# ddemidov/amgcl

Measured on AMD Instinct MI355X. Metric: setup+solve time (s) & iterations to 1e-6, 3D Poisson 512^3, lower is better.
Workload: dtype fp64; 1 GPU; model=3D Poisson 512^3 (7-point stencil), unknowns=134217728, solver=cg, precond=smoothed_aggregation AMG + SPAI0, iters=16, parallelism=single GPU

## Files before the change

### amgcl_amd/csrc/hip/setup.hip

```cpp

#include <hip/hip_runtime.h>

#include <cstdint>

#include "amg_kernels.h"

#define WAVE 64

static inline int nblk(int64_t work, int block = 256, int cap = 4096) {
    int64_t b = (work + block - 1) / block;
    return (int)(b < 1 ? 1 : (b > cap ? cap : b));
}

template <int LANES, int SLOTS>
__device__ __forceinline__ void lds_bitonic(int *k, double *v, int lane) {
    for (int size = 2; size <= SLOTS; size <<= 1) {
        for (int strd = size >> 1; strd > 0; strd >>= 1) {
            __builtin_amdgcn_s_waitcnt(0);
            __builtin_amdgcn_wave_barrier();
            for (int t = lane; t < SLOTS / 2; t += LANES) {
                int i = ((t / strd) * strd * 2) + (t % strd);
                int j = i + strd;
                bool up = ((i & size) == 0);
                int ki = k[i], kj = k[j];
                if ((ki > kj) == up) {
                    k[i] = kj;
                    k[j] = ki;
                    double tv = v[i];
                    v[i] = v[j];
                    v[j] = tv;
                }
            }
        }
    }
    __builtin_amdgcn_s_waitcnt(0);
    __builtin_amdgcn_wave_barrier();
}

__device__ __forceinline__ uint64_t agg_key_d(int i) {
    uint32_t x = (uint32_t)i;
    x ^= x >> 16; x *= 0x7feb352dU; x ^= x >> 15; x *= 0x846ca68bU; x ^= x >> 16;
    return ((uint64_t)x << 32) | (uint32_t)i;
}

#define SETUP_SW 4

__global__ void diag_k(int64_t n, const int *__restrict__ ptr, const int *__restrict__ col,
                       const double *__restrict__ val, double *__restrict__ d) {
    int64_t tid = (int64_t)blockIdx.x * blockDim.x + threadIdx.x;
    int lane = (int)(tid & (SETUP_SW - 1));
    int64_t i = tid / SETUP_SW;
    int64_t stride = ((int64_t)gridDim.x * blockDim.x) / SETUP_SW;
    for (; i < n; i += stride) {
        double v = 0.0;
        for (int j = ptr[i] + lane; j < ptr[i + 1]; j += SETUP_SW)
            if (col[j] == (int)i) v = val[j];
#pragma unroll
        for (int off = SETUP_SW / 2; off > 0; off >>= 1)
            v += __shfl_down(v, off, SETUP_SW);
        if (lane == 0) d[i] = v;
    }
}

__global__ void strong_k(int64_t n, const int *__restrict__ ptr, const int *__restrict__ col,
                         const double *__restrict__ val, const double *__restrict__ d,
                         double eps2, uint8_t *__restrict__ S) {
    int64_t tid = (int64_t)blockIdx.x * blockDim.x + threadIdx.x;
    int lane = (int)(tid & (SETUP_SW - 1));
    int64_t i = tid / SETUP_SW;
    int64_t stride = ((int64_t)gridDim.x * blockDim.x) / SETUP_SW;
    for (; i < n; i += stride) {
        double edi = eps2 * d[i];
        for (int j = ptr[i] + lane; j < ptr[i + 1]; j += SETUP_SW) {
            int c = col[j];
            double v = val[j];
            S[j] = (c != (int)i) && (edi * d[c] < v * v);
        }
    }
}

__global__ void spai0_k(int64_t n, const int *__restrict__ ptr, const int *__restrict__ col,
                        const double *__restrict__ val, double *__restrict__ m) {
    int64_t tid = (int64_t)blockIdx.x * blockDim.x + threadIdx.x;
    int lane = (int)(tid & (SETUP_SW - 1));
    int64_t i = tid / SETUP_SW;
    int64_t stride = ((int64_t)gridDim.x * blockDim.x) / SETUP_SW;
    for (; i < n; i += stride) {
        double num = 0.0, den = 0.0;
        for (int j = ptr[i] + lane; j < ptr[i + 1]; j += SETUP_SW) {
            double v = val[j];
            den += v * v;
            if (col[j] == (int)i) num = v;
        }
#pragma unroll
        for (int off = SETUP_SW / 2; off > 0; off >>= 1) {
            den += __shfl_down(den, off, SETUP_SW);
            num += __shfl_down(num, off, SETUP_SW);
        }
        if (lane == 0) m[i] = den > 0.0 ? num / den : 0.0;
    }
}

extern "C" int amg_setup_diag(int64_t n, const int *ptr, const int *col, const double *val,
                              double *d, hipStream_t s) {
    diag_k<<<nblk(n * SETUP_SW), 256, 0, s>>>(n, ptr, col, val, d);
    return (int)hipGetLastError();
}
extern "C" int amg_setup_strong(int64_t n, const int *ptr, const int *col, const double *val,
                                const double *d, double eps2, uint8_t *S, hipStream_t s) {
    strong_k<<<nblk(n * SETUP_SW), 256, 0, s>>>(n, ptr, col, val, d, eps2, S);
    return (int)hipGetLastError();
}
extern "C" int amg_setup_spai0(int64_t n, const int *ptr, const int *col, const double *val,
                               double *m, hipStream_t s) {
    spai0_k<<<nblk(n * SETUP_SW), 256, 0, s>>>(n, ptr, col, val, m);
    return (int)hipGetLastError();
}

__global__ void gersh_k(int64_t n, const int *__restrict__ ptr, const int *__restrict__ col,
                        const double *__restrict__ val, int scale, double *__restrict__ out) {
    __shared__ double lds[4];
    int64_t i = (int64_t)blockIdx.x * blockDim.x + threadIdx.x;
    int64_t stride = (int64_t)gridDim.x * blockDim.x;
    double m = 0.0;
    for (; i < n; i += stride) {
        double s = 0.0, dia = 1.0;
        for (int j = ptr[i]; j < ptr[i + 1]; ++j) {
            s += fabs(val[j]);
            if (col[j] == (int)i) dia = fabs(val[j]);
        }
        if (scale && dia > 0.0) s /= dia;
        if (s > m) m = s;
    }
#pragma unroll
    for (int off = 32; off > 0; off >>= 1) {
        double o = __shfl_down(m, off, 64);
        if (o > m) m = o;
    }
    int wid = threadIdx.x / 64, lane = threadIdx.x & 63;
    if (lane == 0) lds[wid] = m;
    __syncthreads();
    if (threadIdx.x == 0) {
        double bm = fmax(fmax(lds[0], lds[1]), fmax(lds[2], lds[3]));
        unsigned long long *o = (unsigned long long *)out;
        unsigned long long cur = *o;
        while (__longlong_as_double((long long)cur) < bm) {
            unsigned long long next = (unsigned long long)__double_as_longlong(bm);
            unsigned long long old = atomicCAS(o, cur, next);
            if (old == cur) break;
            cur = old;
        }
    }
}

extern "C" int amg_gershgorin(int64_t n, const int *ptr, const int *col, const double *val,
                              int scale, double *out, hipStream_t s) {
    hipMemsetAsync(out, 0, sizeof(double), s);
    gersh_k<<<nblk(n, 256, 1024), 256, 0, s>>>(n, ptr, col, val, scale, out);
    return (int)hipGetLastError();
}

#define SCAN_BLOCK 1024

__global__ void scan_block_k(int64_t n, const int *__restrict__ in, int *__restrict__ out,
                             int *__restrict__ sums) {
    __shared__ int lds[SCAN_BLOCK];
    int64_t base = (int64_t)blockIdx.x * SCAN_BLOCK;
    int t = threadIdx.x;
    lds[t] = (base + t < n) ? in[base + t] : 0;
    __syncthreads();
    for (int off = 1; off < SCAN_BLOCK; off <<= 1) {
        int v = (t >= off) ? lds[t - off] : 0;
        __syncthreads();
        lds[t] += v;
        __syncthreads();
    }
    if (base + t < n) out[base + t] = lds[t];
    if (t == SCAN_BLOCK - 1 && sums) sums[blockIdx.x] = lds[t];
}

__global__ void scan_add_k(int64_t n, int *__restrict__ out, const int *__restrict__ sums) {
    int64_t base = (int64_t)blockIdx.x * SCAN_BLOCK;
    int t = threadIdx.x;
    if (blockIdx.x > 0 && base + t < n) out[base + t] += sums[blockIdx.x - 1];
}

static int scan_i32_device(int *a, int64_t n, hipStream_t s) {
    if (n <= 0) return 0;
    int64_t nblocks = (n + SCAN_BLOCK - 1) / SCAN_BLOCK;
    if (nblocks == 1) {
        scan_block_k<<<1, SCAN_BLOCK, 0, s>>>(n, a, a, nullptr);
        return (int)hipGetLastError();
    }
    int *sums = nullptr;
    int rc = (int)hipMallocAsync((void **)&sums, nblocks * sizeof(int), s);
    if (rc) return rc;
    scan_block_k<<<nblocks, SCAN_BLOCK, 0, s>>>(n, a, a, sums);
    rc = scan_i32_device(sums, nblocks, s);
    if (rc) return rc;
    scan_add_k<<<nblocks, SCAN_BLOCK, 0, s>>>(n, a, sums);
    hipFreeAsync(sums, s);
    return (int)hipGetLastError();
}

extern "C" int amg_scan_i32(int *a, int64_t n, hipStream_t s) {
    return scan_i32_device(a, n, s);
}

__global__ void agg_init_k(int64_t n, const int *__restrict__ ptr, const uint8_t *__restrict__ S,
                           int *__restrict__ id) {
    int64_t i = (int64_t)blockIdx.x * blockDim.x + threadIdx.x;
    int64_t stride = (int64_t)gridDim.x * blockDim.x;
    for (; i < n; i += stride) {
        int st = -2;
        for (int j = ptr[i]; j < ptr[i + 1]; ++j)
            if (S[j]) { st = -1; break; }
        id[i] = st;
    }
}

#define AGG_FOREACH(i)                                                              int64_t _t = (int64_t)blockIdx.x * blockDim.x + threadIdx.x;                    int64_t _stride = (int64_t)gridDim.x * blockDim.x;                              for (; _t < nwork; _t += _stride)                                                   if (int64_t i = (list ? (int64_t)list[_t] : _t); true)

__global__ void agg_clear_near_k(int64_t nwork, const int *__restrict__ list,
                                 uint8_t *__restrict__ near) {
    AGG_FOREACH(i) near[i] = 0;
}

__global__ void agg_flag_k(int64_t nwork, const int *__restrict__ list,
                           const uint8_t *__restrict__ near, int *__restrict__ flags) {
    AGG_FOREACH(i) flags[_t] = near[i] ? 1 : 0;
}

__global__ void agg_scatter_list_k(int64_t nwork, const int *__restrict__ list,
                                   const uint8_t *__restrict__ near,
                                   const int *__restrict__ flags_scanned,
                                   int *__restrict__ out) {
    AGG_FOREACH(i) if (near[i]) out[flags_scanned[_t] - 1] = (int)i;
}

__global__ void agg_m1_k(int64_t nwork, const int *__restrict__ list,
                         const int *__restrict__ ptr, const int *__restrict__ col,
                         const uint8_t *__restrict__ S, const int *__restrict__ id,
                         const uint8_t *__restrict__ near, uint64_t *__restrict__ m1) {
    AGG_FOREACH(i) {
        if (!near[i]) {
            m1[i] = 0;
            continue;
        }
        uint64_t m = (id[i] == -1) ? agg_key_d((int)i) : 0;
        for (int j = ptr[i]; j < ptr[i + 1]; ++j) {
            if (!S[j]) continue;
            int c = col[j];
            if (id[c] == -1) {
                uint64_t k = agg_key_d(c);
                if (k > m) m = k;
            }
        }
        m1[i] = m;
    }
}

__global__ void agg_near_k(int64_t nwork, const int *__restrict__ list,
                           const int *__restrict__ ptr, const int *__restrict__ col,
                           const uint8_t *__restrict__ S, const int *__restrict__ id,
                           uint8_t *__restrict__ near) {
    AGG_FOREACH(i) {
        if (id[i] == -1) {
            near[i] = 1;
            for (int j = ptr[i]; j < ptr[i + 1]; ++j)
                if (S[j]) near[col[j]] = 1;
        }
    }
}

__global__ void agg_roots_k(int64_t nwork, const int *__restrict__ list,
                            const int *__restrict__ ptr, const int *__restrict__ col,
                            const uint8_t *__restrict__ S, int *__restrict__ id,
                            const uint64_t *__restrict__ m1, uint8_t *__restrict__ newroot) {
    AGG_FOREACH(i) {
        newroot[i] = 0;
        if (id[i] != -1) continue;
        uint64_t key = agg_key_d((int)i);
        uint64_t m2 = m1[i];
        for (int j = ptr[i]; j < ptr[i + 1] && m2 <= key; ++j) {
            if (!S[j]) continue;
            uint64_t v = m1[col[j]];
            if (v > m2) m2 = v;
        }
        if (m2 == key) {
            id[i] = (int)i;
            newroot[i] = 1;
        }
    }
}

__global__ void agg_claim_k(int64_t nwork, const int *__restrict__ list,
                            const int *__restrict__ ptr, const int *__restrict__ col,
                            const uint8_t *__restrict__ S, int *__restrict__ id,
                            uint8_t *__restrict__ prov, const uint8_t *__restrict__ newroot) {
    AGG_FOREACH(i) {
        if (!newroot[i]) continue;
        for (int j = ptr[i]; j < ptr[i + 1]; ++j) {
            int c = col[j];
            if (!S[j]) continue;
            if (id[c] == -1 || prov[c]) {
                id[c] = (int)i;
                prov[c] = 0;
            }
        }
    }
}

__global__ void agg_adopt_mark_k(int64_t nwork, const int *__restrict__ list,
                                 const int *__restrict__ ptr,
                                 const int *__restrict__ col, const uint8_t *__restrict__ S,
                                 const int *__restrict__ id, const uint8_t *__restrict__ prov,
                                 int *__restrict__ choice) {
    AGG_FOREACH(i) {
        if (id[i] != -1) continue;
        uint64_t best = 0;
        int root = -1;
        for (int j = ptr[i]; j < ptr[i + 1]; ++j) {
            int c = col[j];
            if (!S[j] || c == (int)i) continue;
            if (id[c] >= 0 && !prov[c]) {
                uint64_t k = agg_key_d(id[c]);
                if (k > best) { best = k; root = id[c]; }
            }
        }
        choice[i] = root;
    }
}

__global__ void agg_adopt_commit_k(int64_t nwork, const int *__restrict__ list,
                                   int *__restrict__ id,
                                   uint8_t *__restrict__ prov,
                                   const int *__restrict__ choice,
                                   int *__restrict__ remaining) {
    int my_remaining = 0;
    AGG_FOREACH(i) {
        if (id[i] != -1) continue;
        int root = choice[i];
        if (root >= 0) {
            id[i] = root;
            prov[i] = 1;
        } else {
            ++my_remaining;
        }
    }
#pragma unroll
    for (int off = WAVE / 2; off > 0; off >>= 1)
        my_remaining += __shfl_down(my_remaining, off, WAVE);
    if ((threadIdx.x & (WAVE - 1)) == 0 && my_remaining)
        atomicAdd(remaining, my_remaining);
}

__global__ void agg_mark_roots_k(int64_t n, const int *__restrict__ id, int *__restrict__ mark) {
    int64_t i = (int64_t)blockIdx.x * blockDim.x + threadIdx.x;
    int64_t stride = (int64_t)gridDim.x * blockDim.x;
    for (; i < n; i += stride) mark[i] = (id[i] == (int)i) ? 1 : 0;
}

__global__ void agg_relabel_k(int64_t n, int *__restrict__ id, const int *__restrict__ mark) {
    int64_t i = (int64_t)blockIdx.x * blockDim.x + threadIdx.x;
    int64_t stride = (int64_t)gridDim.x * blockDim.x;
    for (; i < n; i += stride)
        if (id[i] >= 0) id[i] = mark[id[i]] - 1;
}

extern "C" int amg_agg_init(int64_t n, const int *ptr, const uint8_t *S, int *id, hipStream_t s) {
    agg_init_k<<<nblk(n), 256, 0, s>>>(n, ptr, S, id);
    return (int)hipGetLastError();
}
static int agg_round_impl(int64_t nwork, const int *list, const int *ptr,
                          const int *col, const uint8_t *S, int *id, uint8_t *prov,
                          uint64_t *m1, uint8_t *newroot, uint8_t *near,
                          int *remaining, hipStream_t s) {
    if (list)
        agg_clear_near_k<<<nblk(nwork), 256, 0, s>>>(nwork, list, near);
    else
        (void)hipMemsetAsync(near, 0, nwork, s);
    agg_near_k<<<nblk(nwork), 256, 0, s>>>(nwork, list, ptr, col, S, id, near);
    agg_m1_k<<<nblk(nwork), 256, 0, s>>>(nwork, list, ptr, col, S, id, near, m1);
    agg_roots_k<<<nblk(nwork), 256, 0, s>>>(nwork, list, ptr, col, S, id, m1, newroot);
    agg_claim_k<<<nblk(nwork), 256, 0, s>>>(nwork, list, ptr, col, S, id, prov, newroot);
    agg_adopt_mark_k<<<nblk(nwork), 256, 0, s>>>(nwork, list, ptr, col, S, id, prov,
                                                 (int *)m1);
    agg_adopt_commit_k<<<nblk(nwork), 256, 0, s>>>(nwork, list, id, prov, (int *)m1,
                                                   remaining);
    return (int)hipGetLastError();
}

extern "C" int amg_agg_round(int64_t n, const int *ptr, const int *col, const uint8_t *S,
                             int *id, uint8_t *prov, uint64_t *m1, uint8_t *newroot,
                             uint8_t *near, int *remaining, hipStream_t s) {
    return agg_round_impl(n, nullptr, ptr, col, S, id, prov, m1, newroot, near,
                          remaining, s);
}
extern "C" int amg_agg_run(int64_t n, const int *ptr, const int *col, const uint8_t *S,
                           int *id, uint8_t *prov, uint64_t *m1, uint8_t *newroot,
                           uint8_t *near, int *remaining, int sync_stride,
                           int max_rounds, int *rounds_out, int *lists,
                           hipStream_t s) {
    int *h_rem = nullptr;
    hipError_t e = hipHostMalloc((void **)&h_rem, 2 * sizeof(int),
                                 hipHostMallocDefault);
    if (e != hipSuccess) return (int)e;
    int *L[2] = {lists, lists ? lists + n : nullptr};
    int cur = -1;
    int64_t nwork = n;
    int64_t last_rem = n;
    int first_cround = -1;
    int rc = 0;
    bool done = false;
    int round = 0;
    for (; round < max_rounds; ++round) {
        e = hipMemsetAsync(remaining, 0, sizeof(int), s);
        if (e != hipSuccess) { rc = (int)e; break; }
        const int *list = cur < 0 ? nullptr : L[cur];
        if (list)
            agg_clear_near_k<<<nblk(nwork), 256, 0, s>>>(nwork, list, near);
        else
            (void)hipMemsetAsync(near, 0, n, s);
        agg_near_k<<<nblk(nwork), 256, 0, s>>>(nwork, list, ptr, col, S, id, near);
        if (lists && last_rem * 4 < n &&
            (first_cround < 0 || (round - first_cround) % 4 == 0)) {
            int nxt = cur < 0 ? 0 : 1 - cur;
            int *F = lists + 2 * n;
            agg_flag_k<<<nblk(nwork), 256, 0, s>>>(nwork, list, near, F);
            rc = scan_i32_device(F, nwork, s);
            if (rc) break;
            agg_scatter_list_k<<<nblk(nwork), 256, 0, s>>>(nwork, list, near, F,
                                                           L[nxt]);
            e = hipMemcpyAsync(h_rem + 1, F + (nwork - 1), sizeof(int),
                               hipMemcpyDeviceToHost, s);
            if (e == hipSuccess) e = hipStreamSynchronize(s);
            if (e != hipSuccess) { rc = (int)e; break; }
            if (h_rem[1] > 0 && h_rem[1] < nwork) {
                cur = nxt;
                nwork = h_rem[1];
            }
            if (first_cround < 0) first_cround = round;
        }
        const int *list2 = cur < 0 ? nullptr : L[cur];
        agg_m1_k<<<nblk(nwork), 256, 0, s>>>(nwork, list2, ptr, col, S, id, near, m1);
        agg_roots_k<<<nblk(nwork), 256, 0, s>>>(nwork, list2, ptr, col, S, id, m1,
                                                newroot);
        agg_claim_k<<<nblk(nwork), 256, 0, s>>>(nwork, list2, ptr, col, S, id, prov,
                                                newroot);
        agg_adopt_mark_k<<<nblk(nwork), 256, 0, s>>>(nwork, list2, ptr, col, S, id,
                                                     prov, (int *)m1);
        agg_adopt_commit_k<<<nblk(nwork), 256, 0, s>>>(nwork, list2, id, prov,
                                                       (int *)m1, remaining);
        rc = (int)hipGetLastError();
        if (rc) break;
        if (round % sync_stride == sync_stride - 1 || round > 8) {
            e = hipMemcpyAsync(h_rem, remaining, sizeof(int), hipMemcpyDeviceToHost, s);
            if (e == hipSuccess) e = hipStreamSynchronize(s);
            if (e != hipSuccess) { rc = (int)e; break; }
            if (*h_rem == 0) { done = true; break; }
            last_rem = *h_rem;
        }
    }
    (void)hipHostFree(h_rem);
    if (rc) return rc;
    if (!done) return 9999;
    if (rounds_out) *rounds_out = round + 1;
    return 0;
}

extern "C" int amg_agg_renumber(int64_t n, int *id, int *mark, hipStream_t s) {
    agg_mark_roots_k<<<nblk(n), 256, 0, s>>>(n, id, mark);
    int rc = scan_i32_device(mark, n, s);
    if (rc) return rc;
    agg_relabel_k<<<nblk(n), 256, 0, s>>>(n, id, mark);
    return (int)hipGetLastError();
}

#define PROW_MAX 56
#define PSLOTS 64
#define PMASK (PSLOTS - 1)
#define PGRP 8

__global__ void psmooth_count_k(int64_t n, const int *__restrict__ ptr,
                                const int *__restrict__ col, const uint8_t *__restrict__ S,
                                const int *__restrict__ id, int *__restrict__ cnt,
                                int *__restrict__ overflow) {
    __shared__ int keys[32][PSLOTS];
    int gid = threadIdx.x / PGRP;
    int lane = threadIdx.x & (PGRP - 1);
    int64_t i = ((int64_t)blockIdx.x * blockDim.x + threadIdx.x) / PGRP;
    int64_t stride = ((int64_t)gridDim.x * blockDim.x) / PGRP;
    int *tk = keys[gid];
    for (; i < n; i += stride) {
        for (int t = lane; t < PSLOTS; t += PGRP) tk[t] = -1;
        __builtin_amdgcn_s_waitcnt(0);
        __builtin_amdgcn_wave_barrier();
        int inserted = 0;
        bool ovf = false;
        for (int j = ptr[i] + lane; j < ptr[i + 1] && !ovf; j += PGRP) {
            int c = col[j];
            if (c != (int)i && !S[j]) continue;
            int a = id[c];
            if (a < 0) continue;
            uint32_t h = ((uint32_t)a * 2654435761u) & PMASK;
            int probes = 0;
            while (true) {
                int old = atomicCAS(&tk[h], -1, a);
                if (old == -1) { ++inserted; break; }
                if (old == a) break;
                h = (h + 1) & PMASK;
                if (++probes >= PSLOTS) { ovf = true; break; }
            }
        }
        if (ovf) atomicAdd(overflow, 1);
#pragma unroll
        for (int off = PGRP / 2; off > 0; off >>= 1)
            inserted += __shfl_down(inserted, off, PGRP);
        if (lane == 0) {
            if (inserted > PROW_MAX) atomicAdd(overflow, 1);
            cnt[i] = inserted;
        }
        __builtin_amdgcn_wave_barrier();
    }
}

__global__ void psmooth_fill_k(int64_t n, const int *__restrict__ ptr,
                               const int *__restrict__ col, const double *__restrict__ val,
                               const uint8_t *__restrict__ S, const int *__restrict__ id,
                               double omega, const int *__restrict__ pptr,
                               int *__restrict__ pcol, double *__restrict__ pval) {
    __shared__ int keys[32][PSLOTS];
    __shared__ double vals[32][PSLOTS];
    int gid = threadIdx.x / PGRP;
    int lane = threadIdx.x & (PGRP - 1);
    int64_t i = ((int64_t)blockIdx.x * blockDim.x + threadIdx.x) / PGRP;
    int64_t stride = ((int64_t)gridDim.x * blockDim.x) / PGRP;
    int *tk = keys[gid];
    double *tv = vals[gid];
    for (; i < n; i += stride) {
        for (int t = lane; t < PSLOTS; t += PGRP) {
            tk[t] = -1;
            tv[t] = 0.0;
        }
        double dia = 0.0;
        for (int j = ptr[i] + lane; j < ptr[i + 1]; j += PGRP)
            if (col[j] == (int)i || !S[j]) dia += val[j];
#pragma unroll
        for (int off = PGRP / 2; off > 0; off >>= 1)
            dia += __shfl_down(dia, off, PGRP);
        dia = __shfl(dia, (threadIdx.x & ~(PGRP - 1)) & 63, 64);
        if (dia != 0.0) dia = -omega / dia;
        __builtin_amdgcn_s_waitcnt(0);
        __builtin_amdgcn_wave_barrier();
        for (int j = ptr[i] + lane; j < ptr[i + 1]; j += PGRP) {
            int c = col[j];
            if (c != (int)i && !S[j]) continue;
            int a = id[c];
            if (a < 0) continue;
            double v = (c == (int)i) ? (1.0 - omega) : dia * val[j];
            uint32_t h = ((uint32_t)a * 2654435761u) & PMASK;
            while (true) {
                int old = atomicCAS(&tk[h], -1, a);
                if (old == -1 || old == a) {
                    atomicAdd(&tv[h], v);
                    break;
                }
                h = (h + 1) & PMASK;
            }
        }
        __builtin_amdgcn_s_waitcnt(0);
        __builtin_amdgcn_wave_barrier();
        int mine = 0;
        for (int t = lane; t < PSLOTS; t += PGRP)
            if (tk[t] != -1) ++mine;
        int off = mine;
#pragma unroll
        for (int d = 1; d < PGRP; d <<= 1) {
            int v = __shfl_up(off, d, PGRP);
            if (lane >= d) off += v;
        }
        off -= mine;
        int base = (i == 0) ? 0 : pptr[i - 1];
        int h2 = base + off;
        for (int t = lane; t < PSLOTS; t += PGRP)
            if (tk[t] != -1) {
                pcol[h2] = tk[t];
                pval[h2] = tv[t];
                ++h2;
            }
        __builtin_amdgcn_wave_barrier();
    }
}

__global__ void ptent_count_k(int64_t n, const int *__restrict__ id, int *__restrict__ cnt) {
    int64_t i = (int64_t)blockIdx.x * blockDim.x + threadIdx.x;
    int64_t stride = (int64_t)gridDim.x * blockDim.x;
    for (; i < n; i += stride) cnt[i] = id[i] >= 0 ? 1 : 0;
}

__global__ void ptent_fill_k(int64_t n, const int *__restrict__ id, const int *__restrict__ pptr,
                             int *__restrict__ pcol, double *__restrict__ pval) {
    int64_t i = (int64_t)blockIdx.x * blockDim.x + threadIdx.x;
    int64_t stride = (int64_t)gridDim.x * blockDim.x;
    for (; i < n; i += stride) {
        if (id[i] < 0) continue;
        int base = (i == 0) ? 0 : pptr[i - 1];
        pcol[base] = id[i];
        pval[base] = 1.0;
    }
}

extern "C" int amg_psmooth_count(int64_t n, const int *ptr, const int *col, const uint8_t *S,
                                 const int *id, int *cnt, int *overflow, hipStream_t s) {
    psmooth_count_k<<<nblk(n * PGRP), 256, 0, s>>>(n, ptr, col, S, id, cnt, overflow);
    return (int)hipGetLastError();
}
extern "C" int amg_psmooth_fill(int64_t n, const int *ptr, const int *col, const double *val,
                                const uint8_t *S, const int *id, double omega,
                                const int *pptr_scanned, int *pcol, double *pval,
                                hipStream_t s) {
    psmooth_fill_k<<<nblk(n * PGRP), 256, 0, s>>>(n, ptr, col, val, S, id, omega,
                                                  pptr_scanned, pcol, pval);
    return (int)hipGetLastError();
}
extern "C" int amg_ptent_count(int64_t n, const int *id, int *cnt, hipStream_t s) {
    ptent_count_k<<<nblk(n), 256, 0, s>>>(n, id, cnt);
    return (int)hipGetLastError();
}
extern "C" int amg_ptent_fill(int64_t n, const int *id, const int *pptr_scanned, int *pcol,
                              double *pval, hipStream_t s) {
    ptent_fill_k<<<nblk(n), 256, 0, s>>>(n, id, pptr_scanned, pcol, pval);
    return (int)hipGetLastError();
}

__global__ void tcount_k(int64_t nnz, const int *__restrict__ col, int *__restrict__ tcnt) {
    int64_t j = (int64_t)blockIdx.x * blockDim.x + threadIdx.x;
    int64_t stride = (int64_t)gridDim.x * blockDim.x;
    for (; j < nnz; j += stride) atomicAdd(&tcnt[col[j]], 1);
}

__global__ void tscatter_k(int64_t n, const int *__restrict__ ptr, const int *__restrict__ col,
                           const double *__restrict__ val, int *__restrict__ cursor,
                           int *__restrict__ tcol, double *__restrict__ tval) {
    int64_t i = (int64_t)blockIdx.x * blockDim.x + threadIdx.x;
    int64_t stride = (int64_t)gridDim.x * blockDim.x;
    for (; i < n; i += stride) {
        for (int j = ptr[i]; j < ptr[i + 1]; ++j) {
            int c = col[j];
            int h = atomicAdd(&cursor[c], 1);
            tcol[h] = (int)i;
            tval[h] = val[j];
        }
    }
}

__global__ void sort_rows_k(int64_t n, const int *__restrict__ ptr_scanned,
                            int *__restrict__ col, double *__restrict__ val) {
    int64_t i = (int64_t)blockIdx.x * blockDim.x + threadIdx.x;
    int64_t stride = (int64_t)gridDim.x * blockDim.x;
    for (; i < n; i += stride) {
        int b = (i == 0) ? 0 : ptr_scanned[i - 1];
        int e = ptr_scanned[i];
        for (int k = b + 1; k < e; ++k) {
            int ck = col[k];
            double vk = val[k];
            int m = k;
            while (m > b && col[m - 1] > ck) {
                col[m] = col[m - 1];
                val[m] = val[m - 1];
                --m;
            }
            col[m] = ck;
            val[m] = vk;
        }
    }
}

extern "C" int amg_transpose_count(int64_t nnz, const int *col, int *tcnt, hipStream_t s) {
    tcount_k<<<nblk(nnz), 256, 0, s>>>(nnz, col, tcnt);
    return (int)hipGetLastError();
}
extern "C" int amg_transpose_scatter(int64_t n, const int *ptr, const int *col,
                                     const double *val, int *cursor, int *tcol, double *tval,
                                     hipStream_t s) {
    tscatter_k<<<nblk(n), 256, 0, s>>>(n, ptr, col, val, cursor, tcol, tval);
    return (int)hipGetLastError();
}
extern "C" int amg_sort_rows(int64_t n, const int *ptr_scanned, int *col, double *val,
                             hipStream_t s) {
    sort_rows_k<<<nblk(n), 256, 0, s>>>(n, ptr_scanned, col, val);
    return (int)hipGetLastError();
}

#define HSLOTS 512
#define HMASK (HSLOTS - 1)
#define SGRP 8
#define SSLOTS 128
#define SSMASK (SSLOTS - 1)
#define SGSMALL 96

__global__ void spgemm_ub_k(int64_t an, const int *__restrict__ aptr,
                            const int *__restrict__ acol, const int *__restrict__ bptr,
                            int *__restrict__ ub) {
    int64_t i = (int64_t)blockIdx.x * blockDim.x + threadIdx.x;
    int64_t stride = (int64_t)gridDim.x * blockDim.x;
    for (; i < an; i += stride) {
        int u = 0;
        for (int ja = aptr[i]; ja < aptr[i + 1]; ++ja) {
            int ca = acol[ja];
            u += bptr[ca + 1] - bptr[ca];
        }
        ub[i] = u;
    }
}

template <int SLOTS>
__global__ void spgemm_count_small_k(int64_t an, const int *__restrict__ aptr,
                                     const int *__restrict__ acol,
                                     const int *__restrict__ bptr,
                                     const int *__restrict__ bcol,
                                     const int *__restrict__ ub, int *__restrict__ cnt,
                                     int ub_lo, int ub_hi) {
    __shared__ int keys[32][SLOTS];
    constexpr int MASK = SLOTS - 1;
    int gid = threadIdx.x / SGRP;
    int lane = threadIdx.x & (SGRP - 1);
    int64_t row = ((int64_t)blockIdx.x * blockDim.x + threadIdx.x) / SGRP;
    int64_t stride = ((int64_t)gridDim.x * blockDim.x) / SGRP;
    int *tk = keys[gid];
    for (; row < an; row += stride) {
        int u = ub[row];
        if (u <= ub_lo || u > ub_hi) continue;
        for (int t = lane; t < SLOTS; t += SGRP) tk[t] = -1;
        __builtin_amdgcn_s_waitcnt(0);
        __builtin_amdgcn_wave_barrier();
        int inserted = 0;
        for (int ja = aptr[row]; ja < aptr[row + 1]; ++ja) {
            int ca = acol[ja];
            for (int jb = bptr[ca] + lane; jb < bptr[ca + 1]; jb += SGRP) {
                int key = bcol[jb];
                uint32_t h = ((uint32_t)key * 2654435761u) & MASK;
                while (true) {
                    int old = atomicCAS(&tk[h], -1, key);
                    if (old == -1) { ++inserted; break; }
                    if (old == key) break;
                    h = (h + 1) & MASK;
                }
            }
        }
#pragma unroll
        for (int off = SGRP / 2; off > 0; off >>= 1)
            inserted += __shfl_down(inserted, off, SGRP);
        if (lane == 0) cnt[row] = inserted;
        __builtin_amdgcn_wave_barrier();
    }
}

template <int SLOTS>
__global__ void spgemm_fill_small_k(int64_t an, const int *__restrict__ aptr,
                                    const int *__restrict__ acol,
                                    const double *__restrict__ aval,
                                    const int *__restrict__ bptr,
                                    const int *__restrict__ bcol,
                                    const double *__restrict__ bval,
                                    const int *__restrict__ ub,
                                    const int *__restrict__ cptr_scanned,
                                    int *__restrict__ ccol, double *__restrict__ cval,
                                    int do_sort, int len_lo, int len_hi) {
    __shared__ int keys[32][SLOTS];
    __shared__ double vals[32][SLOTS];
    constexpr int SMASK_S = SLOTS - 1;
    int gid = threadIdx.x / SGRP;
    int lane = threadIdx.x & (SGRP - 1);
    int64_t row = ((int64_t)blockIdx.x * blockDim.x + threadIdx.x) / SGRP;
    int64_t stride = ((int64_t)gridDim.x * blockDim.x) / SGRP;
    int *tk = keys[gid];
    double *tv = vals[gid];
    for (; row < an; row += stride) {
        if (ub[row] > SGSMALL) continue;
        int base = (row == 0) ? 0 : cptr_scanned[row - 1];
        int len = cptr_scanned[row] - base;
        if (len <= len_lo || len > len_hi) continue;
        for (int t = lane; t < SLOTS; t += SGRP) {
            tk[t] = -1;
            tv[t] = 0.0;
        }
        __builtin_amdgcn_s_waitcnt(0);
        __builtin_amdgcn_wave_barrier();
        for (int ja = aptr[row]; ja < aptr[row + 1]; ++ja) {
            int ca = acol[ja];
            double va = aval[ja];
            for (int jb = bptr[ca] + lane; jb < bptr[ca + 1]; jb += SGRP) {
                int key = bcol[jb];
                double v = va * bval[jb];
                uint32_t h = ((uint32_t)key * 2654435761u) & SMASK_S;
                while (true) {
                    int old = atomicCAS(&tk[h], -1, key);
                    if (old == -1 || old == key) {
                        atomicAdd(&tv[h], v);
                        break;
                    }
                    h = (h + 1) & SMASK_S;
                }
            }
        }
        __builtin_amdgcn_s_waitcnt(0);
        __builtin_amdgcn_wave_barrier();
        if (do_sort) {
            for (int t = lane; t < SLOTS; t += SGRP)
                if (tk[t] == -1) tk[t] = 0x7fffffff;
            lds_bitonic<SGRP, SLOTS>(tk, tv, lane);
            for (int t = lane; t < len; t += SGRP) {
                ccol[base + t] = tk[t];
                cval[base + t] = tv[t];
            }
        } else {
            int mine = 0;
            for (int t = lane; t < SLOTS; t += SGRP)
                if (tk[t] != -1) ++mine;
            int off = mine;
#pragma unroll
            for (int d = 1; d < SGRP; d <<= 1) {
                int v = __shfl_up(off, d, SGRP);
                if (lane >= d) off += v;
            }
            off -= mine;
            int h = base + off;
            for (int t = lane; t < SLOTS; t += SGRP)
                if (tk[t] != -1) {
                    ccol[h] = tk[t];
                    cval[h] = tv[t];
                    ++h;
                }
        }
        __builtin_amdgcn_wave_barrier();
    }
}

#define BIGROW 256

__device__ __forceinline__ int pfx_find(const int *pfx, int len, int t) {
    int lo = 0, hi = len;
    while (hi - lo > 1) {
        int mid = (lo + hi) >> 1;
        if (pfx[mid] <= t) lo = mid;
        else hi = mid;
    }
    return lo;
}

__global__ void spg_bigflag_k(int64_t an, const int *__restrict__ ub,
                              int *__restrict__ flags) {
    int64_t i = (int64_t)blockIdx.x * blockDim.x + threadIdx.x;
    int64_t stride = (int64_t)gridDim.x * blockDim.x;
    for (; i < an; i += stride) flags[i] = ub[i] > SGSMALL ? 1 : 0;
}

__global__ void spg_bigscatter_k(int64_t an, const int *__restrict__ ub,
                                 const int *__restrict__ flags_scanned,
                                 int *__restrict__ list, int *__restrict__ nbig) {
    int64_t i = (int64_t)blockIdx.x * blockDim.x + threadIdx.x;
    int64_t stride = (int64_t)gridDim.x * blockDim.x;
    for (; i < an; i += stride) {
        if (ub[i] > SGSMALL) list[flags_scanned[i] - 1] = (int)i;
        if (i == an - 1) *nbig = flags_scanned[i];
    }
}

template <int SLOTS>
__global__ void spgemm_count_k(int64_t an, const int *__restrict__ biglist,
                               const int *__restrict__ nbig,
                               const int *__restrict__ aptr,
                               const int *__restrict__ acol, const int *__restrict__ bptr,
                               const int *__restrict__ bcol, const int *__restrict__ ub,
                               int *__restrict__ cnt, int *__restrict__ overflow,
                               int ub_lo, int ub_hi) {
    __shared__ int keys[4][SLOTS];
    __shared__ int pfx[4][BIGROW + 1];
    __shared__ int bbeg[4][BIGROW];
    constexpr int SMASK = SLOTS - 1;
    int wid = threadIdx.x / WAVE;
    int lane = threadIdx.x & (WAVE - 1);
    int64_t idx = ((int64_t)blockIdx.x * blockDim.x + threadIdx.x) / WAVE;
    int64_t stride = ((int64_t)gridDim.x * blockDim.x) / WAVE;
    const int64_t nwork = *nbig;
    int *tk = keys[wid];

    for (; idx < nwork; idx += stride) {
        int64_t row = biglist[idx];
        int total = ub[row];
        if (total <= ub_lo || total > ub_hi) continue;
        int ab = aptr[row], alen = aptr[row + 1] - ab;
        for (int t = lane; t < SLOTS; t += WAVE) tk[t] = -1;
        const bool huge = alen > BIGROW;
        if (!huge && lane == 0) {
            int acc = 0;
            for (int j = 0; j < alen; ++j) {
                pfx[wid][j] = acc;
                int ca = acol[ab + j];
                bbeg[wid][j] = bptr[ca];
                acc += bptr[ca + 1] - bptr[ca];
            }
            pfx[wid][alen] = acc;
        }
        __builtin_amdgcn_s_waitcnt(0);
        __builtin_amdgcn_wave_barrier();
        int inserted = 0;
        bool ovf = false;
        if (huge) {
            for (int j = 0; j < alen && !ovf; ++j) {
                int ca = acol[ab + j];
                for (int jb = bptr[ca] + lane; jb < bptr[ca + 1] && !ovf;
                     jb += WAVE) {
                    int key = bcol[jb];
                    uint32_t h = ((uint32_t)key * 2654435761u) & SMASK;
                    int probes = 0;
                    while (true) {
                        int old = atomicCAS(&tk[h], -1, key);
                        if (old == -1) { ++inserted; break; }
                        if (old == key) break;
                        h = (h + 1) & SMASK;
                        if (++probes >= SLOTS) { ovf = true; break; }
                    }
                }
            }
        } else {
        for (int t = lane; t < total && !ovf; t += WAVE) {
            int ja = pfx_find(pfx[wid], alen, t);
            int key = bcol[bbeg[wid][ja] + (t - pfx[wid][ja])];
            uint32_t h = ((uint32_t)key * 2654435761u) & SMASK;
            int probes = 0;
            while (true) {
                int old = atomicCAS(&tk[h], -1, key);
                if (old == -1) { ++inserted; break; }
                if (old == key) break;
                h = (h + 1) & SMASK;
                if (++probes >= SLOTS) { ovf = true; break; }
            }
        }
        }
        if (ovf && lane == 0) atomicAdd(overflow, 1);
#pragma unroll
        for (int off = WAVE / 2; off > 0; off >>= 1)
            inserted += __shfl_down(inserted, off, WAVE);
        if (lane == 0) cnt[row] = inserted;
        __builtin_amdgcn_wave_barrier();
    }
}

#define MIDLEN 96

template <int SLOTS>
__global__ void spgemm_fill_k(int64_t an, const int *__restrict__ biglist,
                              const int *__restrict__ nbig,
                              const int *__restrict__ aptr,
                              const int *__restrict__ acol, const double *__restrict__ aval,
                              const int *__restrict__ bptr, const int *__restrict__ bcol,
                              const double *__restrict__ bval, const int *__restrict__ ub,
                              const int *__restrict__ cptr_scanned, int *__restrict__ ccol,
                              double *__restrict__ cval, int do_sort, int len_lo,
                              int len_hi) {
    __shared__ int keys[4][SLOTS];
    __shared__ double vals[4][SLOTS];
    __shared__ int pfx[4][BIGROW + 1];
    __shared__ int bbeg[4][BIGROW];
    __shared__ double av[4][BIGROW];
    constexpr int SMASK = SLOTS - 1;
    int wid = threadIdx.x / WAVE;
    int lane = threadIdx.x & (WAVE - 1);
    int64_t idx = ((int64_t)blockIdx.x * blockDim.x + threadIdx.x) / WAVE;
    int64_t stride = ((int64_t)gridDim.x * blockDim.x) / WAVE;
    const int64_t nwork = *nbig;
    int *tk = keys[wid];
    double *tv = vals[wid];

    for (; idx < nwork; idx += stride) {
        int64_t row = biglist[idx];
        int total = ub[row];
        if (total <= SGSMALL) continue;
        int ab = aptr[row], alen = aptr[row + 1] - ab;
        int base = (row == 0) ? 0 : cptr_scanned[row - 1];
        int len = cptr_scanned[row] - base;
        if (len <= len_lo || len > len_hi) continue;
        const bool huge = alen > BIGROW;
        for (int t = lane; t < SLOTS; t += WAVE) {
            tk[t] = -1;
            tv[t] = 0.0;
        }
        if (!huge) {
            for (int j = lane; j < alen; j += WAVE) av[wid][j] = aval[ab + j];
            if (lane == 0) {
                int acc = 0;
                for (int j = 0; j < alen; ++j) {
                    pfx[wid][j] = acc;
                    int ca = acol[ab + j];
                    bbeg[wid][j] = bptr[ca];
                    acc += bptr[ca + 1] - bptr[ca];
                }
                pfx[wid][alen] = acc;
            }
        }
        __builtin_amdgcn_s_waitcnt(0);
        __builtin_amdgcn_wave_barrier();
        if (huge) {
            for (int j = 0; j < alen; ++j) {
                int ca = acol[ab + j];
                double va = aval[ab + j];
                for (int jb = bptr[ca] + lane; jb < bptr[ca + 1]; jb += WAVE) {
                    int key = bcol[jb];
                    double v = va * bval[jb];
                    uint32_t h = ((uint32_t)key * 2654435761u) & SMASK;
                    while (true) {
                        int old = atomicCAS(&tk[h], -1, key);
                        if (old == -1 || old == key) {
                            atomicAdd(&tv[h], v);
                            break;
                        }
                        h = (h + 1) & SMASK;
                    }
                }
            }
        } else {
        for (int t = lane; t < total; t += WAVE) {
            int ja = pfx_find(pfx[wid], alen, t);
            int jb = bbeg[wid][ja] + (t - pfx[wid][ja]);
            int key = bcol[jb];
            double v = av[wid][ja] * bval[jb];
            uint32_t h = ((uint32_t)key * 2654435761u) & SMASK;
            while (true) {
                int old = atomicCAS(&tk[h], -1, key);
                if (old == -1 || old == key) {
                    atomicAdd(&tv[h], v);
                    break;
                }
                h = (h + 1) & SMASK;
            }
        }
        }
        __builtin_amdgcn_s_waitcnt(0);
        __builtin_amdgcn_wave_barrier();
        if (do_sort) {
            for (int t = lane; t < SLOTS; t += WAVE)
                if (tk[t] == -1) tk[t] = 0x7fffffff;
            lds_bitonic<WAVE, SLOTS>(tk, tv, lane);
            for (int t = lane; t < len; t += WAVE) {
                ccol[base + t] = tk[t];
                cval[base + t] = tv[t];
            }
        } else {
            int mine = 0;
            for (int t = lane; t < SLOTS; t += WAVE)
                if (tk[t] != -1) ++mine;
            int off = mine;
#pragma unroll
            for (int d = 1; d < WAVE; d <<= 1) {
                int v = __shfl_up(off, d, WAVE);
                if (lane >= d) off += v;
            }
            off -= mine;
            int h = base + off;
            for (int t = lane; t < SLOTS; t += WAVE)
                if (tk[t] != -1) {
                    ccol[h] = tk[t];
                    cval[h] = tv[t];
                    ++h;
                }
        }
        __builtin_amdgcn_wave_barrier();
    }
}

__global__ void poisson_cnt_k(int64_t n, int64_t nz, int64_t row_beg, int64_t row_end,
                              int *__restrict__ cnt) {
    int64_t idx = row_beg + (int64_t)blockIdx.x * blockDim.x + threadIdx.x;
    int64_t stride = (int64_t)gridDim.x * blockDim.x;
    for (; idx < row_end; idx += stride) {
        int64_t i = idx % n, j = (idx / n) % n, k = idx / (n * n);
        cnt[idx - row_beg] =
            1 + (k > 0) + (j > 0) + (i > 0) + (i + 1 < n) + (j + 1 < n) + (k + 1 < nz);
    }
}

__global__ void poisson_fill_k(int64_t n, int64_t nz, int64_t row_beg, int64_t row_end,
                               const int *__restrict__ ptr_scanned,
                               int *__restrict__ col, double *__restrict__ val) {
    int64_t idx = row_beg + (int64_t)blockIdx.x * blockDim.x + threadIdx.x;
    int64_t stride = (int64_t)gridDim.x * blockDim.x;
    for (; idx < row_end; idx += stride) {
        int64_t i = idx % n, j = (idx / n) % n, k = idx / (n * n);
        int64_t loc = idx - row_beg;
        int h = (loc == 0) ? 0 : ptr_scanned[loc - 1];
        if (k > 0)      { col[h] = (int)(idx - n * n); val[h] = -1.0; ++h; }
        if (j > 0)      { col[h] = (int)(idx - n);     val[h] = -1.0; ++h; }
        if (i > 0)      { col[h] = (int)(idx - 1);     val[h] = -1.0; ++h; }
        col[h] = (int)idx; val[h] = 6.0; ++h;
        if (i + 1 < n)  { col[h] = (int)(idx + 1);     val[h] = -1.0; ++h; }
        if (j + 1 < n)  { col[h] = (int)(idx + n);     val[h] = -1.0; ++h; }
        if (k + 1 < nz) { col[h] = (int)(idx + n * n); val[h] = -1.0; ++h; }
    }
}

extern "C" int amg_poisson_cnt(int64_t n, int64_t nz, int64_t row_beg, int64_t row_end,
                               int *cnt, hipStream_t s) {
    poisson_cnt_k<<<nblk(row_end - row_beg), 256, 0, s>>>(n, nz, row_beg, row_end, cnt);
    return (int)hipGetLastError();
}
extern "C" int amg_poisson_fill(int64_t n, int64_t nz, int64_t row_beg, int64_t row_end,
                                const int *ptr_scanned, int *col, double *val,
                                hipStream_t s) {
    poisson_fill_k<<<nblk(row_end - row_beg), 256, 0, s>>>(n, nz, row_beg, row_end,
                                                           ptr_scanned, col, val);
    return (int)hipGetLastError();
}

extern "C" int amg_spgemm_count(int64_t an, const int *aptr, const int *acol, const int *bptr,
                                const int *bcol, int *ub, int *cnt, int *overflow,
                                int *bigscratch, hipStream_t s) {
    int *flags = bigscratch;
    int *biglist = bigscratch + an;
    int *nbig = bigscratch + 2 * an;
    spgemm_ub_k<<<nblk(an), 256, 0, s>>>(an, aptr, acol, bptr, ub);
    spg_bigflag_k<<<nblk(an), 256, 0, s>>>(an, ub, flags);
    int rc = scan_i32_device(flags, an, s);
    if (rc) return rc;
    spg_bigscatter_k<<<nblk(an), 256, 0, s>>>(an, ub, flags, biglist, nbig);
    spgemm_count_small_k<SSLOTS><<<nblk(an * SGRP), 256, 0, s>>>(
        an, aptr, acol, bptr, bcol, ub, cnt, 0, SGSMALL);
    spgemm_count_k<HSLOTS><<<nblk(an * WAVE), 256, 0, s>>>(
        an, biglist, nbig, aptr, acol, bptr, bcol, ub, cnt, overflow, SGSMALL, 1 << 30);
    return (int)hipGetLastError();
}
extern "C" int amg_spgemm_fill(int64_t an, const int *aptr, const int *acol, const double *aval,
                               const int *bptr, const int *bcol, const double *bval,
                               const int *ub, const int *cptr_scanned, int *ccol,
                               double *cval, int do_sort, const int *bigscratch,
                               hipStream_t s) {
    const int *biglist = bigscratch + an;
    const int *nbig = bigscratch + 2 * an;
    spgemm_fill_small_k<32><<<nblk(an * SGRP), 256, 0, s>>>(an, aptr, acol, aval, bptr,
                                                            bcol, bval, ub, cptr_scanned,
                                                            ccol, cval, do_sort, 0, 20);
    spgemm_fill_small_k<64><<<nblk(an * SGRP), 256, 0, s>>>(an, aptr, acol, aval, bptr,
                                                            bcol, bval, ub, cptr_scanned,
                                                            ccol, cval, do_sort, 20, 48);
    spgemm_fill_small_k<SSLOTS><<<nblk(an * SGRP), 256, 0, s>>>(an, aptr, acol, aval, bptr,
                                                                bcol, bval, ub, cptr_scanned,
                                                                ccol, cval, do_sort, 48,
                                                                1 << 30);
    spgemm_fill_k<128><<<nblk(an * WAVE), 256, 0, s>>>(
        an, biglist, nbig, aptr, acol, aval, bptr, bcol, bval, ub, cptr_scanned, ccol,
        cval, do_sort, 0, MIDLEN);
    spgemm_fill_k<HSLOTS><<<nblk(an * WAVE), 256, 0, s>>>(
        an, biglist, nbig, aptr, acol, aval, bptr, bcol, bval, ub, cptr_scanned, ccol,
        cval, do_sort, MIDLEN, 1 << 30);
    return (int)hipGetLastError();
}
```

Baseline: 893.6 ms.

## Parallelize SpGEMM row expansion with subgroup scans and load-balanced flattening

In the small-row count kernel, lanes now load A-row entries cooperatively, prefix-scan the B-row lengths and flatten the product into a single load-balanced index space. This replaces the nested per-A-entry loop, where short B rows left most lanes idle. The small-row fill kernel preloads A entries across lanes and broadcasts them by shuffle. In the big-row kernels, the serial lane-0 prefix build is replaced by a wave-wide scan. In exchange the count path does more shuffle and select work per element (a fully unrolled SGRP-step search), and results change only in atomic accumulation order.

```diff
diff --git a/amgcl_amd/csrc/hip/setup.hip b/amgcl_amd/csrc/hip/setup.hip
--- a/amgcl_amd/csrc/hip/setup.hip
+++ b/amgcl_amd/csrc/hip/setup.hip
@@ -715,6 +715,27 @@
     }
 }
 
+__device__ __forceinline__ int sg_scan(int x, int lane) {
+#pragma unroll
+    for (int d = 1; d < SGRP; d <<= 1) {
+        int v = __shfl_up(x, d, SGRP);
+        if (lane >= d) x += v;
+    }
+    return x;
+}
+
+__device__ __forceinline__ int sg_find(const int (&p)[SGRP], int t, int &e) {
+    int ja = 0;
+    e = 0;
+#pragma unroll
+    for (int k = 0; k < SGRP - 1; ++k)
+        if (p[k] <= t) {
+            ja = k + 1;
+            e = p[k];
+        }
+    return ja;
+}
+
 template <int SLOTS>
 __global__ void spgemm_count_small_k(int64_t an, const int *__restrict__ aptr,
                                      const int *__restrict__ acol,
@@ -736,16 +757,33 @@
         __builtin_amdgcn_s_waitcnt(0);
         __builtin_amdgcn_wave_barrier();
         int inserted = 0;
-        for (int ja = aptr[row]; ja < aptr[row + 1]; ++ja) {
-            int ca = acol[ja];
-            for (int jb = bptr[ca] + lane; jb < bptr[ca + 1]; jb += SGRP) {
-                int key = bcol[jb];
-                uint32_t h = ((uint32_t)key * 2654435761u) & MASK;
-                while (true) {
-                    int old = atomicCAS(&tk[h], -1, key);
-                    if (old == -1) { ++inserted; break; }
-                    if (old == key) break;
-                    h = (h + 1) & MASK;
+        const int aend = aptr[row + 1];
+        for (int j0 = aptr[row]; j0 < aend; j0 += SGRP) {
+            int j = j0 + lane;
+            int bb = 0, bl = 0;
+            if (j < aend) {
+                int ca = acol[j];
+                bb = bptr[ca];
+                bl = bptr[ca + 1] - bb;
+            }
+            int inc = sg_scan(bl, lane);
+            int p[SGRP];
+#pragma unroll
+            for (int k = 0; k < SGRP; ++k) p[k] = __shfl(inc, k, SGRP);
+            const int tot = p[SGRP - 1];
+            for (int t0 = 0; t0 < tot; t0 += SGRP) {
+                int t = t0 + lane, e;
+                int ja = sg_find(p, t, e);
+                int bj = __shfl(bb, ja, SGRP);
+                if (t < tot) {
+                    int key = bcol[bj + (t - e)];
+                    uint32_t h = ((uint32_t)key * 2654435761u) & MASK;
+                    while (true) {
+                        int old = atomicCAS(&tk[h], -1, key);
+                        if (old == -1) { ++inserted; break; }
+                        if (old == key) break;
+                        h = (h + 1) & MASK;
+                    }
                 }
             }
         }
@@ -788,20 +826,34 @@
         }
         __builtin_amdgcn_s_waitcnt(0);
         __builtin_amdgcn_wave_barrier();
-        for (int ja = aptr[row]; ja < aptr[row + 1]; ++ja) {
-            int ca = acol[ja];
-            double va = aval[ja];
-            for (int jb = bptr[ca] + lane; jb < bptr[ca + 1]; jb += SGRP) {
-                int key = bcol[jb];
-                double v = va * bval[jb];
-                uint32_t h = ((uint32_t)key * 2654435761u) & SMASK_S;
-                while (true) {
-                    int old = atomicCAS(&tk[h], -1, key);
-                    if (old == -1 || old == key) {
-                        atomicAdd(&tv[h], v);
-                        break;
+        const int aend = aptr[row + 1];
+        for (int j0 = aptr[row]; j0 < aend; j0 += SGRP) {
+            int j = j0 + lane;
+            int bb = 0, bl = 0;
+            double va = 0.0;
+            if (j < aend) {
+                int ca = acol[j];
+                va = aval[j];
+                bb = bptr[ca];
+                bl = bptr[ca + 1] - bb;
+            }
+            const int nj = min(SGRP, aend - j0);
+            for (int k = 0; k < nj; ++k) {
+                const int bk = __shfl(bb, k, SGRP);
+                const int ek = bk + __shfl(bl, k, SGRP);
+                const double vk = __shfl(va, k, SGRP);
+                for (int jb = bk + lane; jb < ek; jb += SGRP) {
+                    int key = bcol[jb];
+                    double v = vk * bval[jb];
+                    uint32_t h = ((uint32_t)key * 2654435761u) & SMASK_S;
+                    while (true) {
+                        int old = atomicCAS(&tk[h], -1, key);
+                        if (old == -1 || old == key) {
+                            atomicAdd(&tv[h], v);
+                            break;
+                        }
+                        h = (h + 1) & SMASK_S;
                     }
-                    h = (h + 1) & SMASK_S;
                 }
             }
         }
@@ -848,6 +900,15 @@
         else hi = mid;
     }
     return lo;
+}
+
+__device__ __forceinline__ int wave_scan(int x, int lane) {
+#pragma unroll
+    for (int d = 1; d < WAVE; d <<= 1) {
+        int v = __shfl_up(x, d, WAVE);
+        if (lane >= d) x += v;
+    }
+    return x;
 }
 
 __global__ void spg_bigflag_k(int64_t an, const int *__restrict__ ub,
@@ -894,15 +955,24 @@
         int ab = aptr[row], alen = aptr[row + 1] - ab;
         for (int t = lane; t < SLOTS; t += WAVE) tk[t] = -1;
         const bool huge = alen > BIGROW;
-        if (!huge && lane == 0) {
+        if (!huge) {
             int acc = 0;
-            for (int j = 0; j < alen; ++j) {
-                pfx[wid][j] = acc;
-                int ca = acol[ab + j];
-                bbeg[wid][j] = bptr[ca];
-                acc += bptr[ca + 1] - bptr[ca];
-            }
-            pfx[wid][alen] = acc;
+            for (int j0 = 0; j0 < alen; j0 += WAVE) {
+                int j = j0 + lane;
+                int bb = 0, bl = 0;
+                if (j < alen) {
+                    int ca = acol[ab + j];
+                    bb = bptr[ca];
+                    bl = bptr[ca + 1] - bb;
+                }
+                int inc = wave_scan(bl, lane);
+                if (j < alen) {
+                    pfx[wid][j] = acc + inc - bl;
+                    bbeg[wid][j] = bb;
+                }
+                acc += __shfl(inc, WAVE - 1, WAVE);
+            }
+            if (lane == 0) pfx[wid][alen] = acc;
         }
         __builtin_amdgcn_s_waitcnt(0);
         __builtin_amdgcn_wave_barrier();
@@ -989,17 +1059,24 @@
             tv[t] = 0.0;
         }
         if (!huge) {
-            for (int j = lane; j < alen; j += WAVE) av[wid][j] = aval[ab + j];
-            if (lane == 0) {
-                int acc = 0;
-                for (int j = 0; j < alen; ++j) {
-                    pfx[wid][j] = acc;
+            int acc = 0;
+            for (int j0 = 0; j0 < alen; j0 += WAVE) {
+                int j = j0 + lane;
+                int bb = 0, bl = 0;
+                if (j < alen) {
                     int ca = acol[ab + j];
-                    bbeg[wid][j] = bptr[ca];
-                    acc += bptr[ca + 1] - bptr[ca];
+                    av[wid][j] = aval[ab + j];
+                    bb = bptr[ca];
+                    bl = bptr[ca + 1] - bb;
                 }
-                pfx[wid][alen] = acc;
-            }
+                int inc = wave_scan(bl, lane);
+                if (j < alen) {
+                    pfx[wid][j] = acc + inc - bl;
+                    bbeg[wid][j] = bb;
+                }
+                acc += __shfl(inc, WAVE - 1, WAVE);
+            }
+            if (lane == 0) pfx[wid][alen] = acc;
         }
         __builtin_amdgcn_s_waitcnt(0);
         __builtin_amdgcn_wave_barrier();
```

After: 832.0 ms (median of 6 runs). 1.07x faster.
